# acerbilab/gpyreg

Hardware: AMD Instinct MI355X
Metric: GP-fits/sec (NLL+grad, N=4096 D=10) (higher is better)
Workload: dtype f64

## Files before the change

gpyreg_amd/_lib.py:

```python

from __future__ import annotations

import ctypes as C
import os
import threading

import numpy as np

_HERE = os.path.dirname(os.path.abspath(__file__))
LIB_PATH = os.environ.get("GPYREG_AMD_LIB") or os.path.join(_HERE, "lib", "libgpcore.so")

K_SE, K_MATERN, K_RQ, K_SE_ISO, K_MATERN_ISO = range(5)
F64, F32 = 0, 1
KLO_ZERO, KLO_ROW, KLO_COL = 0, 1, 2
KHI_FULL, KHI_ROW, KHI_COL = 0, 1, 2

_dp = C.c_void_p
_ip = C.c_void_p
_vp = C.c_void_p
_dpp = C.POINTER(C.c_double)

SIGNATURES = {
    "gpc_create": (C.c_int, [C.c_int, C.POINTER(_vp)]),
    "gpc_destroy": (None, [_vp]),
# ... 334 lines not shown
    @_serial
    def last_lauum_timing(self):
        a, b = C.c_double(), C.c_double()
        self._lib.gpc_last_lauum_timing(self._h, C.byref(a), C.byref(b))
        return a.value, b.value

    @_serial
    def mfma_peak(self, dtype=F64):
        t, cyc, ghz = C.c_double(), C.c_double(), C.c_double()
        rc = self._lib.gpc_mfma_peak(self._h, dtype, C.byref(t), C.byref(cyc), C.byref(ghz))
        self._check(rc, "gpc_mfma_peak")
        return t.value, cyc.value, ghz.value

    @_serial
    def debug_gemm(self, A, B, Cm, M, N, K, a_kmajor, b_kmajor, alpha=1.0, beta=0, klo=0, khi=0,
                   lower_only=False, dtype=F64, force_bt=0):
        A, B = _f64(A), _f64(B)
        Cm = _f64(Cm).copy()
        flags = int(bool(lower_only)) | {0: 0, 64: 0x100, 128: 0x200, 12864: 0x400}[force_bt]
        rc = self._lib.gpc_debug_gemm(self._h, dtype, M, N, K, int(a_kmajor), int(b_kmajor),
                                      float(alpha), int(beta), klo, khi, flags, _ptr(A),
                                      _ptr(B), _ptr(Cm))
        self._check(rc, "gpc_debug_gemm")
        return Cm

    @_serial
    def debug_factor(self, A, want_inv=True, dtype=F64):
        A = _f64(A)
        n = A.shape[0]
        L, W = np.empty((n, n)), np.empty((n, n))
        Ainv = np.empty((n, n)) if want_inv else None
        logdet = C.c_double()
        info = C.c_int()
        rc = self._lib.gpc_debug_factor(self._h, dtype, n, _ptr(A), _ptr(L), _ptr(W), _ptr(Ainv),
# ... 295 lines not shown
```

gpyreg_amd/csrc/gemm.h:

```cpp
#pragma once
#include "common.h"

#include <type_traits>

namespace gpc {

template <typename T>
constexpr int BKT_v = sizeof(T) == 4 ? 32 : 16;
template <typename T>
constexpr bool MM_SWZ = sizeof(T) == 4;
template <typename T>
constexpr int LDQ_v = MM_SWZ<T> ? BKT_v<T> : BKT_v<T> + 1;
constexpr int ldp_of(int BT) { return BT + 16; }
template <typename T>
constexpr int opsz_of(int BT) {
  return BKT_v<T> * (BT + 16) > BT * LDQ_v<T> ? BKT_v<T> * (BT + 16) : BT * LDQ_v<T>;
}

enum { KLO_ZERO = 0, KLO_ROW = 1, KLO_COL = 2 };
enum { KHI_FULL = 0, KHI_ROW = 1, KHI_COL = 2 };

struct GemmArgs {
  const void* A;
  const void* B;
  void* C;
  long long sA, sB, sC;
  int lda, ldb, ldc;
  int M, N, K;
  double alpha;
  int beta;
  int klo, khi, lower_only;
  int tiles_m, tiles_n;
  int flags = 0;
  const unsigned short* rsv = nullptr;
  int* ctr = nullptr;
  int ntiles = 0, batch = 0;
  double* colsq = nullptr;
  const double* ep_w = nullptr;
  long long ep_sw = 0;
  const double* ep_alpha = nullptr;
};
inline int g_gemm_flags = 8 | 16;

template <typename T, bool KM, int BT, int NT>
__device__ __forceinline__ unsigned stage_toff(int ld, int t) {
  constexpr int VEC = MM<T>::VEC;
  if constexpr (!KM) {
    constexpr int TPR = BKT_v<T> / VEC;
    return (unsigned)(t / TPR) * (unsigned)ld + (unsigned)((t % TPR) * VEC);
  } else {
    constexpr int VPR = BT / VEC;
    return (unsigned)(t / VPR) * (unsigned)ld + (unsigned)((t % VPR) * VEC);
  }
}
template <typename T, bool KM, int BT, int NT>
__device__ __forceinline__ size_t stage_pstride(int ld) {
// ... 460 lines not shown
    if (nsq <= 0) continue;
    const int total = ((g.ntiles - cls + nclass - 1) / nclass) * nsq;
    for (;;) {
      if (threadIdx.x == 0) next_tile = atomicAdd(g.ctr + q, 1);
      __syncthreads();
      const int idx = __builtin_amdgcn_readfirstlane(next_tile);
      __syncthreads();
      if (idx >= total) break;
      const int ntq = total / nsq;
      const int sq = idx / ntq, tq = idx - sq * ntq;
      gemm_tile<T, AKM, BKM, BT, NW, 0, EPI>(g, cls + tq * nclass, smp + NQ * sq, smem);
    }
  }
}

inline int g_persist_spare = 0;
inline long long g_gemm_launches = 0;
inline int g_block_slots = 512;
template <typename T, int BT, int NW>
inline hipError_t launch_gemm_bt(hipStream_t st, GemmArgs g, bool akm, bool bkm, int batch, int* ctr = nullptr,
                                 const unsigned short* reserve = nullptr) {
  const int tm = g.M / BT, tn = g.N / BT;
  g.tiles_m = tm;
  g.tiles_n = tn;
  g.flags = g_gemm_flags;
  const int ntiles = g.lower_only ? tm * (tm + 1) / 2 : tm * tn;
  if (ntiles <= 0 || batch <= 0) return hipSuccess;
  ++g_gemm_launches;
  g.ntiles = ntiles;
  g.batch = batch;
  g.ctr = ctr;
  const unsigned dyn = 0u;
  const int cap = (BT == 128 ? g_block_slots : 2 * g_block_slots) - g_persist_spare;
  g.rsv = reserve;
  if (ctr && (BT == 128 || reserve) && cap > 0 && ((long long)ntiles * batch > cap || reserve)) {
    dim3 grid(reserve ? (BT == 128 ? cap + 96 : cap) : cap), block(64 * NW);
    if (!akm && !bkm)
      hipLaunchKernelGGL((gemm_persist_kernel<T, false, false, BT, NW>), grid, block, dyn, st, g);
    else if (!akm && bkm)
      hipLaunchKernelGGL((gemm_persist_kernel<T, false, true, BT, NW>), grid, block, dyn, st, g);
    else if (akm && bkm)
      hipLaunchKernelGGL((gemm_persist_kernel<T, true, true, BT, NW>), grid, block, dyn, st, g);
    else
      hipLaunchKernelGGL((gemm_persist_kernel<T, true, false, BT, NW>), grid, block, dyn, st, g);
    return hipGetLastError();
  }
  dim3 grid(ntiles, batch), block(64 * NW);
  if (!akm && !bkm)
    hipLaunchKernelGGL((gemm_kernel<T, false, false, BT, NW>), grid, block, dyn, st, g);
  else if (!akm && bkm)
    hipLaunchKernelGGL((gemm_kernel<T, false, true, BT, NW>), grid, block, dyn, st, g);
  else if (akm && bkm)
    hipLaunchKernelGGL((gemm_kernel<T, true, true, BT, NW>), grid, block, dyn, st, g);
  else
    hipLaunchKernelGGL((gemm_kernel<T, true, false, BT, NW>), grid, block, dyn, st, g);
  return hipGetLastError();
}

#ifdef GPC_EXPERIMENTS
template <typename T>
inline hipError_t launch_gemm_rect(hipStream_t st, GemmArgs g, bool akm, bool bkm, int batch) {
  constexpr int BT = 128, BTN = 64;
// ... 78 lines not shown
  constexpr int BT = 64;
  int n[2];
  GemmArgs* gs[2] = {&g1, &g2};
  for (int i = 0; i < 2; ++i) {
    GemmArgs& g = *gs[i];
    g.tiles_m = g.M / BT;
    g.tiles_n = g.N / BT;
    g.flags = g_gemm_flags;
    g.ntiles = n[i] = g.lower_only ? g.tiles_m * (g.tiles_m + 1) / 2 : g.tiles_m * g.tiles_n;
    g.batch = batch;
    g.ctr = nullptr;
    g.rsv = nullptr;
  }
  if (n[0] + n[1] <= 0 || batch <= 0) return hipSuccess;
  ++g_gemm_launches;
  hipLaunchKernelGGL((gemm_dual_kernel<T, false, false, false, true, BT, 4>), dim3(n[0] + n[1], batch), dim3(256), 0, st,
                     g1, g2, n[0]);
  return hipGetLastError();
}

template <typename T>
inline hipError_t launch_gemm_colsq(hipStream_t st, GemmArgs g, int batch, int* ctr) {
  constexpr int BT = 128;
  g.tiles_m = g.M / BT;
  g.tiles_n = g.N / BT;
  g.flags = g_gemm_flags;
  g.lower_only = 0;
  g.ntiles = g.tiles_m * g.tiles_n;
  if (g.ntiles <= 0 || batch <= 0) return hipSuccess;
  ++g_gemm_launches;
// ... 44 lines not shown
```

gpyreg_amd/csrc/gpcore.hip:

```cpp
#include "../../include/gpcore.h"

#include <algorithm>
#include <atomic>
#include <chrono>
#include <cmath>
#include <cstdlib>
#include <cstring>
#include <memory>
#include <mutex>

#include "blas1.h"
#include "block_append.h"
#include "common.h"
#include "covfun.h"
#include "draw.h"
#include "gemm.h"
#include "leaf.h"
#include "lookahead.h"
#include "plan.h"
#include "quad.h"
#include "quad_mix.h"
#ifdef GPC_EXPERIMENTS
#include "dag.h"
#endif
// ... 2877 lines not shown
  g.A = c->dbg1.p;
  g.B = c->dbg2.p;
  g.C = c->dbg3.p;
  g.sA = g.sB = g.sC = 0;
  g.lda = akm ? M : K;
  g.ldb = bkm ? N : K;
  g.ldc = N;
  g.M = M;
  g.N = N;
  g.K = K;
  g.alpha = alpha;
  g.beta = beta;
  g.klo = klo;
  g.khi = khi;
  g.lower_only = lower & 1;
  g.tiles_n = N / TILE;
  HIPCHK(c, launch_gemm<T>(c->st, g, akm != 0, bkm != 0, 1, (lower & 0x100) ? 64 : ((lower & 0x200) ? 128 : ((lower & 0x400) ? 12864 : 0))));
  return download_as<T>(c, c->dbg3.as<T>(), C, (size_t)M * N);
}

template <typename T>
int debug_factor_impl(gpc_ctx* c, int n, const double* A, double* L, double* W, double* Ainv,
                      double* logdet, int* info) {
  const int npad = pad_tile(n);
  const size_t msz = (size_t)npad * npad;
  HIPCHK(c, c->mA.ensure(msz * sizeof(T)));
  HIPCHK(c, c->mW.ensure(msz * sizeof(T)));
  HIPCHK(c, c->mT.ensure(msz * sizeof(T)));
  HIPCHK(c, c->dbg1.ensure((size_t)n * n * 8));
  HIPCHK(c, c->scal.ensure(64));
  HIPCHK(c, hipMemcpyAsync(c->dbg1.p, A, (size_t)n * n * 8, hipMemcpyHostToDevice, c->st));
  HIPCHK(c, hipMemsetAsync(c->scal.p, 0, 64, c->st));
// ... 872 lines not shown
    g_create_err = "probing the CU map failed: " + c->err;
    delete c;
    return -1;
  }
  if (const char* e = getenv("GPC_LEAF")) gpc::g_leaf_version = atoi(e) == 3 ? 3 : 5;
  if (const char* e = getenv("GPC_SMALL_PATH")) c->small_path = atoi(e) != 0;
  if (const char* e = getenv("GPC_GRAPH_MAX_NPAD")) c->graph_max_npad = atoi(e);
#ifdef GPC_EXPERIMENTS
  if (const char* e = getenv("GPC_RL_PANEL")) c->rl_panel = atoi(e) <= 0 ? 0 : std::max(TILE, (atoi(e) / TILE) * TILE);
  if (const char* e = getenv("GPC_RECT_MIN")) gpc::g_rect_min_blocks = atoi(e);
#endif
  if (const char* e = getenv("GPC_NLL_BLOCK")) c->nll_block = atoi(e) < 0 ? -1 : (atoi(e) == 0 ? 0 : std::max(TILE, (atoi(e) / TILE) * TILE));
  if (const char* e = getenv("GPC_GROUPS")) c->groups = std::max(1, std::min((int)gpc_ctx::MAXG, atoi(e)));
  if (const char* e = getenv("GPC_SMALL_BLOCKS")) gpc::g_small_launch_blocks = atoi(e);
  if (const char* e = getenv("GPC_DUAL")) gpc::g_dual_launch = atoi(e) != 0;
  if (const char* e = getenv("GPC_GEMM_FLAGS")) gpc::g_gemm_flags = atoi(e);
  if (const char* e = getenv("GPC_XCD_AFFINE")) gpc::g_gemm_flags = atoi(e) ? (gpc::g_gemm_flags | 8) : (gpc::g_gemm_flags & ~8);
  *out = c;
  return 0;
}

void gpc_destroy(gpc_ctx* c) {
  if (!c) return;
  (void)hipSetDevice(c->device);
  (void)hipStreamSynchronize(c->st);
  DevBuf* bufs[] = {&c->dX,   &c->dY,  &c->mA,    &c->mW,  &c->mT,   &c->xs,   &c->spb,  &c->mulb, &c->divb,
                    &c->dvec, &c->rvec,  &c->zvec, &c->avec, &c->scal, &c->parts, &c->gout, &c->diagq,
                    &c->dmb,  &c->dsn2b, &c->mg,  &c->ng,   &c->ks,   &c->vb,   &c->xss,  &c->pout, &c->kss,
                    &c->dbg1, &c->dbg2,  &c->dbg3, &c->tpart, &c->qb, &c->gpart, &c->gres, &c->qcon, &c->qmix, &c->zb, &c->fb, &c->dout, &c->daux, &c->tile_ctr, &c->rsv_tbl};
  for (auto& g : c->graphs)
// ... 634 lines not shown
  if (n == "dag_timeout_ms") return std::max(1, value);
  return value;
}
#endif
}

int gpc_set_option(gpc_ctx* c, const char* name, int value) {
  if (!c || !name) return -2;
  const std::string n(name);
  if (n == "groups")
    c->groups = std::max(1, std::min((int)gpc_ctx::MAXG, value));
  else if (n == "small_blocks")
    gpc::g_small_launch_blocks = value;
  else if (n == "dual_launch")
    gpc::g_dual_launch = value != 0;
  else if (n == "leaf")
    gpc::g_leaf_version = value == 3 ? 3 : 5;
  else if (n == "defer_min")
    c->defer_min = value;
  else if (n == "defer_reserve") {
    c->defer_reserve = value;
    if (build_reserve_table(c)) return -1;
  } else if (n == "leaf_fault")
    gpc::g_leaf_fault = value != 0;
  else if (n == "nll_block")
    c->nll_block = value < 0 ? -1 : (value == 0 ? 0 : std::max(TILE, (value / TILE) * TILE));
  else if (n == "solves_beside_lauum")
    c->solves_beside_lauum = value != 0;
  else if (n == "stable")
    c->stable = value != 0;
// ... 17 lines not shown
      *slot = clamp_experiment_option(n, value);
    else
#endif
      FAIL(c, "gpc_set_option: unknown option");
  }
  ++g_alloc_epoch;
  return 0;
}

int gpc_get_option(gpc_ctx* c, const char* name, int* value) {
  if (!c || !name || !value) return -2;
  const std::string n(name);
  if (n == "groups") *value = c->groups;
  else if (n == "small_blocks") *value = gpc::g_small_launch_blocks;
  else if (n == "dual_launch") *value = gpc::g_dual_launch ? 1 : 0;
  else if (n == "leaf") *value = gpc::g_leaf_version;
  else if (n == "defer_min") *value = c->defer_min;
  else if (n == "defer_reserve") *value = c->defer_reserve;
  else if (n == "nll_block") *value = c->nll_block;
  else if (n == "solves_beside_lauum") *value = c->solves_beside_lauum;
  else if (n == "stable") *value = c->stable;
  else if (n == "small_path") *value = c->small_path;
  else if (n == "check_queues") *value = c->check_queues;
  else if (n == "small_poll") *value = c->small_poll;
  else if (n == "small_timing") *value = c->small_timing;
  else if (n == "small_polled") *value = (int)(c->small_polled & 0x7fffffff);
  else if (n == "small_synced") *value = (int)(c->small_synced & 0x7fffffff);
  else if (n == "cov_fused") *value = (int)(c->cov_fused & 0x7fffffff);
  else if (n == "quad_mix_gemms") *value = (int)(c->quad_mix_gemms & 0x7fffffff);
  else if (n == "block_engine") *value = c->block_engine;
// ... 100 lines not shown
        best_cyc = best_ghz * 1e9 * (4.0 * prop.multiProcessorCount) * (2.0 * 16 * 16 * 4) / (tf * 1e12);
      }
    }
  *tflops = best;
  if (cycles_per_mfma) *cycles_per_mfma = best_cyc;
  if (clock_ghz) *clock_ghz = best_ghz;
  return 0;
}


int gpc_debug_gemm(gpc_ctx* c, int dtype, int M, int N, int K, int a_kmajor, int b_kmajor, double alpha,
                   int beta, int klo, int khi, int lower_only, const double* A, const double* B, double* C) {
  if (!c) return -2;
  if (M % TILE || N % TILE || K % TILE || M <= 0 || N <= 0 || K <= 0) FAIL(c, "gpc_debug_gemm: sizes must be multiples of 128");
  if ((lower_only & 1) && M != N) FAIL(c, "gpc_debug_gemm: lower_only needs M == N");
#ifndef GPC_EXPERIMENTS
  if (lower_only & 0x400) FAIL(c, "gpc_debug_gemm: the rectangular tile exists in the experiments build only");
#endif
  HIPCHK(c, hipSetDevice(c->device));
  return dtype == GPC_F64
             ? debug_gemm_impl<double>(c, M, N, K, a_kmajor, b_kmajor, alpha, beta, klo, khi, lower_only, A, B, C)
             : debug_gemm_impl<float>(c, M, N, K, a_kmajor, b_kmajor, alpha, beta, klo, khi, lower_only, A, B, C);
}

int gpc_debug_leaf(gpc_ctx* c, int dtype, const double* A, double* L, double* W, double* logdet, int* info) {
  return gpc_debug_factor(c, dtype, TILE, A, L, W, nullptr, logdet, info);
}

int gpc_debug_factor(gpc_ctx* c, int dtype, int n, const double* A, double* L, double* W, double* Ainv,
                     double* logdet, int* info) {
// ... 112 lines not shown
```

gpyreg_amd/csrc/plan.h:

```cpp
#pragma once
#include "blas1.h"
#include "gemm.h"
#include "leaf.h"

#include <algorithm>

namespace gpc {

#ifdef GPC_EXPERIMENTS
struct PlanRecorder {
  struct Op {
    int kind;
    GemmArgs g;
    bool akm, bkm;
    int off;
  };
  std::vector<Op> ops;
  bool unsupported = false;
};
#endif

template <typename T>
struct Factor {
#ifdef GPC_EXPERIMENTS
// ... 36 lines not shown
  hipEvent_t ev_tail = nullptr;
  int tail_row0 = 1 << 30;
  void need_rows(int hi) {
    if (ev_tail && hi > tail_row0) {
      chk(hipStreamWaitEvent(st, ev_tail, 0));
      ev_tail = nullptr;
    }
  }
  double flops = 0;
  int launches = 0;
  hipError_t err = hipSuccess;

  T* blk(T* base, int r, int c) const { return base + (size_t)r * npad + c; }

  GemmArgs make_args(T* C, long long sC, const T* Aop, long long sAop, const T* Bop, long long sBop, int M, int N,
                     int K, double alpha, int beta, int klo, int khi, int lower) {
    GemmArgs g;
    g.A = Aop;
    g.B = Bop;
    g.C = C;
    g.sA = sAop;
    g.sB = sBop;
    g.sC = sC;
    g.lda = g.ldb = g.ldc = npad;
    g.M = M;
    g.N = N;
    g.K = K;
    g.alpha = alpha;
    g.beta = beta;
    g.klo = klo;
    g.khi = khi;
    g.lower_only = lower;
    g.tiles_n = N / TILE;
    flops += gemm_flops(g, batch);
    return g;
  }

  void gemm(T* C, long long sC, const T* Aop, long long sAop, const T* Bop, long long sBop, int M,
            int N, int K, bool akm, bool bkm, double alpha, int beta, int klo, int khi, int lower,
            hipStream_t on = nullptr, const unsigned short* rsv = nullptr) {
    GemmArgs g;
    g.A = Aop;
    g.B = Bop;
    g.C = C;
    g.sA = sAop;
    g.sB = sBop;
    g.sC = sC;
    g.lda = g.ldb = g.ldc = npad;
    g.M = M;
    g.N = N;
    g.K = K;
    g.alpha = alpha;
    g.beta = beta;
    g.klo = klo;
    g.khi = khi;
    g.lower_only = lower;
    g.tiles_n = N / TILE;
    flops += gemm_flops(g, batch);
    ++launches;
#ifdef GPC_EXPERIMENTS
    if (rec) {
      rec->ops.push_back({0, g, akm, bkm, 0});
      return;
    }
#endif
    int* slot = nullptr;
    const long long tm = M / TILE, tn = N / TILE;
    const long long blocks128 = (lower ? tm * (tm + 1) / 2 : tm * tn) * batch;
    if (!rsv && reserve_all && reserve && blocks128 >= reserve_min) rsv = reserve;
    const bool persistent = rsv || (blocks128 >= g_small_launch_blocks && blocks128 > g_block_slots - g_persist_spare);
    if (persistent && ctr && ctr_used + CTR_STRIDE <= ctr_cap) {
// ... 22 lines not shown
      }
#endif
      need_rows(off + TILE);
      launch_leaf<T>(st, batch, blk(A, off, off), sA, npad, blk(W, off, off), sW, npad, off, logdet, info,
                     std::max(0, std::min(TILE, nvalid - off)), stable);
      flops += (2.0 / 3.0) * TILE * (double)TILE * TILE * batch;
      ++launches;
      return;
    }
    const int q = n / TILE;
    const int n1 = (q / 2) * TILE, n2 = n - n1;
    const int o1 = off, o2 = off + n1;
    potrf_inv(o1, n1, true, keep_L);
    need_rows(o2 + n2);
    gemm(blk(Tm, o2, o1), sT, blk(A, o2, o1), sA, blk(W, o1, o1), sW, n2, n1, n1, false, false, 1.0,
         0, KLO_ZERO, KHI_COL, 0);
    if (stable) {
      gemm(blk(A, o2, o1), sA, blk(Tm, o2, o1), sT, blk(A, o1, o1), sA, n2, n1, n1, false, false, -1.0, 1, KLO_ZERO,
           KHI_COL, 0);
      gemm(blk(Tm, o2, o1), sT, blk(A, o2, o1), sA, blk(W, o1, o1), sW, n2, n1, n1, false, false, 1.0, 1, KLO_ZERO,
           KHI_COL, 0);
    }
    const bool defer = need_inv && side && defer_min > 0 && n >= defer_min && ev_used + 2 <= nev;
    bool u_done = false;
    {
      GemmArgs gs = make_args(blk(A, o2, o2), sA, blk(Tm, o2, o1), sT, blk(Tm, o2, o1), sT, n2, n2, n1, -1.0, 1,
                              KLO_ZERO, KHI_FULL, 1);
      const long long syrk_tiles = (long long)(n2 / TILE) * (n2 / TILE + 1) / 2 * batch;
      if (need_inv && !defer && dual_launch && !rec && gemm_is_small(gs, batch) && !(reserve_all && syrk_tiles >= reserve_min)) {
        GemmArgs gu = make_args(blk(A, o2, o1), sA, blk(Tm, o2, o1), sT, blk(W, o1, o1), sW, n2, n1, n1, 1.0, 0,
                                KLO_COL, KHI_FULL, 0);
        if (gemm_is_small(gu, batch)) {
          hipError_t e = launch_gemm_dual_small<T>(st, gs, gu, batch);
          if (e != hipSuccess && err == hipSuccess) err = e;
          ++launches;
          u_done = true;
        } else {
          flops -= gemm_flops(gu, batch);
        }
      }
      if (!u_done) {
        flops -= gemm_flops(gs, batch);
        gemm(blk(A, o2, o2), sA, blk(Tm, o2, o1), sT, blk(Tm, o2, o1), sT, n2, n2, n1, false, false, -1.0, 1,
             KLO_ZERO, KHI_FULL, 1);
      }
    }
    hipEvent_t ev_join = nullptr;
    if (defer) {
      hipEvent_t ev_fork = evs[ev_used++];
      ev_join = evs[ev_used++];
      chk(hipEventRecord(ev_fork, st));
      chk(hipStreamWaitEvent(side, ev_fork, 0));
      gemm(blk(A, o2, o1), sA, blk(Tm, o2, o1), sT, blk(W, o1, o1), sW, n2, n1, n1, false, true, 1.0, 0,
           KLO_COL, KHI_FULL, 0, side, reserve);
      chk(hipEventRecord(ev_join, side));
    }
    potrf_inv(o2, n2, need_inv, keep_L);
    if (need_inv) {
      if (defer)
        chk(hipStreamWaitEvent(st, ev_join, 0));
      else if (!u_done)
        gemm(blk(A, o2, o1), sA, blk(Tm, o2, o1), sT, blk(W, o1, o1), sW, n2, n1, n1, false, true, 1.0, 0,
             KLO_COL, KHI_FULL, 0);
      gemm(blk(W, o2, o1), sW, blk(W, o2, o2), sW, blk(A, o2, o1), sA, n2, n1, n2, false, true, -1.0,
           0, KLO_ZERO, KHI_ROW, 0);
    }
#ifdef GPC_EXPERIMENTS
    if (keep_L && rec) rec->unsupported = true;
#endif
    if (keep_L && !rec) {
      dim3 grid((n1 + 64 * MM<T>::VEC - 1) / (64 * MM<T>::VEC), n2 / 32, batch), block(64, 4);
      hipLaunchKernelGGL((rect_copy_kernel<T>), grid, block, 0, st, (const T*)blk(Tm, o2, o1), sT, npad,
                         blk(A, o2, o1), sA, npad, n2, n1);
      ++launches;
    }
  }

  int nll_block = 0;

  void trsm_nll(int r0, int m, int c0, int n) {
    if (n <= nll_block) {
      gemm(blk(Tm, r0, c0), sT, blk(A, r0, c0), sA, blk(W, c0, c0), sW, m, n, n, false, false, 1.0, 0, KLO_ZERO,
           KHI_COL, 0);
      if (stable) {
        gemm(blk(A, r0, c0), sA, blk(Tm, r0, c0), sT, blk(A, c0, c0), sA, m, n, n, false, false, -1.0, 1, KLO_ZERO,
             KHI_COL, 0);
        gemm(blk(Tm, r0, c0), sT, blk(A, r0, c0), sA, blk(W, c0, c0), sW, m, n, n, false, false, 1.0, 1, KLO_ZERO,
             KHI_COL, 0);
      }
      return;
    }
    const int q = n / TILE;
    const int n1 = (q / 2) * TILE, n2 = n - n1;
    trsm_nll(r0, m, c0, n1);
    gemm(blk(A, r0, c0 + n1), sA, blk(Tm, r0, c0), sT, blk(Tm, c0 + n1, c0), sT, m, n2, n1, false, false, -1.0, 1,
         KLO_ZERO, KHI_FULL, 0);
    trsm_nll(r0, m, c0 + n1, n2);
  }

  void potrf_nll(int off, int n) {
    if (n <= nll_block || n == TILE) {
      potrf_inv(off, n, true, false);
      return;
    }
    const int q = n / TILE;
    const int n1 = (q / 2) * TILE, n2 = n - n1;
    const int o1 = off, o2 = off + n1;
    potrf_nll(o1, n1);
    need_rows(o2 + n2);
    trsm_nll(o2, n2, o1, n1);
    gemm(blk(A, o2, o2), sA, blk(Tm, o2, o1), sT, blk(Tm, o2, o1), sT, n2, n2, n1, false, false, -1.0, 1, KLO_ZERO,
         KHI_FULL, 1);
    potrf_nll(o2, n2);
  }

  void forward_solve_nll(int off, int n, double* r, double* z) {
    if (n <= nll_block || n == TILE) {
      hipLaunchKernelGGL((trmv_kernel<T>), dim3(n / 4, batch), dim3(256), 0, st, (const T*)W, sW, npad,
                         (const double*)r, npad, z, off);
      ++launches;
      return;
    }
    const int q = n / TILE;
    const int n1 = (q / 2) * TILE, n2 = n - n1;
    forward_solve_nll(off, n1, r, z);
    hipLaunchKernelGGL((gemv_sub_kernel<T>), dim3(n2 / 4, batch), dim3(256), 0, st, (const T*)Tm, sT, npad,
                       (const double*)z, r, npad, off + n1, off, n1);
// ... 67 lines not shown
        hipLaunchKernelGGL((trmv_kernel<T>), dim3(n / 4, batch), dim3(256), 0, st, (const T*)W, sW, npad,
                           (const double*)r, npad, z, off);
      ++launches;
      return;
    }
    const int q = n / TILE;
    const int n1 = (q / 2) * TILE, n2 = n - n1;
    forward_solve(off, n1, true, r, z);
    hipLaunchKernelGGL((gemv_sub_kernel<T>), dim3(n2 / 4, batch), dim3(256), 0, st, (const T*)Tm, sT, npad,
                       (const double*)z, r, npad, off + n1, off, n1);
    ++launches;
    forward_solve(off + n1, n2, need_inv, r, z);
  }

  void lauum(T* out, long long sOut) {
    gemm(out, sOut, W, sW, W, sW, npad, npad, npad, true, true, 1.0, 0, KLO_ROW, KHI_FULL, 1);
  }
};

}
```

Before: 839.5.

## Add triangle-aware GEMM kernels that skip zero MFMA blocks in edge slabs

```diff
diff --git a/gpyreg_amd/_lib.py b/gpyreg_amd/_lib.py
--- a/gpyreg_amd/_lib.py
+++ b/gpyreg_amd/_lib.py
@@ -372,10 +372,11 @@
 
     @_serial
     def debug_gemm(self, A, B, Cm, M, N, K, a_kmajor, b_kmajor, alpha=1.0, beta=0, klo=0, khi=0,
-                   lower_only=False, dtype=F64, force_bt=0):
+                   lower_only=False, dtype=F64, force_bt=0, tri=0, batch=1):
         A, B = _f64(A), _f64(B)
         Cm = _f64(Cm).copy()
         flags = int(bool(lower_only)) | {0: 0, 64: 0x100, 128: 0x200, 12864: 0x400}[force_bt]
+        flags |= (int(tri) & 15) << 12 | (int(batch) & 0xff) << 16
         rc = self._lib.gpc_debug_gemm(self._h, dtype, M, N, K, int(a_kmajor), int(b_kmajor),
                                       float(alpha), int(beta), klo, khi, flags, _ptr(A),
                                       _ptr(B), _ptr(Cm))
diff --git a/gpyreg_amd/csrc/gemm.h b/gpyreg_amd/csrc/gemm.h
--- a/gpyreg_amd/csrc/gemm.h
+++ b/gpyreg_amd/csrc/gemm.h
@@ -19,6 +19,7 @@
 
 enum { KLO_ZERO = 0, KLO_ROW = 1, KLO_COL = 2 };
 enum { KHI_FULL = 0, KHI_ROW = 1, KHI_COL = 2 };
+enum { TRI_NONE = 0, TRI_A_FIRST = 1, TRI_A_LAST = 2, TRI_B_FIRST = 3, TRI_B_LAST = 4, TRI_OPND = 7, TRI_SYM = 8 };
 
 struct GemmArgs {
   const void* A;
@@ -39,7 +40,9 @@
   const double* ep_w = nullptr;
   long long ep_sw = 0;
   const double* ep_alpha = nullptr;
+  int tri = TRI_NONE;
 };
+inline int g_tri_skip = 1;
 inline int g_gemm_flags = 8 | 16;
 
 template <typename T, bool KM, int BT, int NT>
@@ -530,6 +533,373 @@
   }
 }
 
+template <int ILO, int IHI, int JLO, int JHI, bool DG = false>
+struct Live {
+  static constexpr int ilo = ILO, ihi = IHI, jlo = JLO, jhi = JHI;
+  static constexpr bool on(int i, int j) { return i >= ILO && i < IHI && j >= JLO && j < JHI && (!DG || i >= j); }
+  static constexpr int count() {
+    int n = 0;
+    for (int i = ILO; i < IHI; ++i)
+      for (int j = JLO; j < JHI; ++j) n += on(i, j) ? 1 : 0;
+    return n;
+  }
+};
+
+template <bool AKM, bool BKM, int BT, int TRI, bool DG>
+__device__ __forceinline__ void gemm_tile_tri_at(const GemmArgs& g, const int ti, const int tj, const int by,
+                                                 double* __restrict__ smem) {
+  using T = double;
+  using acc_t = typename MM<T>::acc_t;
+  using vec_t = typename MM<T>::vec_t;
+  constexpr int NT = 256, BK = BKT_v<T>;
+  constexpr int NV = (BT * BK) / (NT * MM<T>::VEC);
+  constexpr int OPSZ = opsz_of<T>(BT), STG = 2 * OPSZ;
+  constexpr int MR = BT / 32;
+  constexpr int TOP = TRI & TRI_OPND;
+  static_assert(TRI != TRI_NONE && NV >= 1 && MR >= 2 && (!DG || (TRI & TRI_SYM)), "tile shape");
+  const int t = threadIdx.x;
+  const int lane = t & 63, w = t >> 6, wr = w >> 1, wc = w & 1;
+  const int m0 = ti * BT, n0 = tj * BT;
+  int k0 = g.klo == KLO_ROW ? m0 : (g.klo == KLO_COL ? n0 : 0);
+  int k1 = g.khi == KHI_ROW ? m0 + BT : (g.khi == KHI_COL ? n0 + BT : g.K);
+  if (k1 > g.K) k1 = g.K;
+  const int nk = (k1 - k0) / BK;
+
+  const T* __restrict__ A = reinterpret_cast<const T*>(g.A) + (size_t)by * g.sA;
+  const T* __restrict__ B = reinterpret_cast<const T*>(g.B) + (size_t)by * g.sB;
+  T* __restrict__ C = reinterpret_cast<T*>(g.C) + (size_t)by * g.sC;
+
+  acc_t acc[MR][MR];
+#pragma unroll
+  for (int i = 0; i < MR; ++i)
+#pragma unroll
+    for (int j = 0; j < MR; ++j) acc[i][j] = acc_t{0, 0, 0, 0};
+
+  if (nk > 0) {
+    vec_t ra[NV], rb[NV];
+    const unsigned toa = stage_toff<T, AKM, BT, NT>(g.lda, t) * (unsigned)sizeof(T),
+                   tob = stage_toff<T, BKM, BT, NT>(g.ldb, t) * (unsigned)sizeof(T);
+    const unsigned psa = (unsigned)(stage_pstride<T, AKM, BT, NT>(g.lda) * sizeof(T)),
+                   psb = (unsigned)(stage_pstride<T, BKM, BT, NT>(g.ldb) * sizeof(T));
+    const T* pa = AKM ? A + (size_t)k0 * g.lda + m0 : A + (size_t)m0 * g.lda + k0;
+    const T* pb = BKM ? B + (size_t)k0 * g.ldb + n0 : B + (size_t)n0 * g.ldb + k0;
+    const size_t rowsa = (size_t)BK * g.lda, rowsb = (size_t)BK * g.ldb;
+    __amdgpu_buffer_rsrc_t rsa = make_rsrc(pa), rsb = make_rsrc(pb);
+    unsigned ua = 0, ub = 0;
+    auto next_slab = [&]() {
+      if constexpr (AKM) {
+        pa += rowsa;
+        rsa = make_rsrc(pa);
+      } else {
+        ua += (unsigned)(BK * sizeof(T));
+      }
+      if constexpr (BKM) {
+        pb += rowsb;
+        rsb = make_rsrc(pb);
+      } else {
+        ub += (unsigned)(BK * sizeof(T));
+      }
+    };
+    g2r<T, AKM, BT, NT>(ra, rsa, ua, psa, toa);
+    g2r<T, BKM, BT, NT>(rb, rsb, ub, psb, tob);
+    r2s<T, AKM, BT, NT>(smem, ra, t);
+    r2s<T, BKM, BT, NT>(smem + OPSZ, rb, t);
+    next_slab();
+    g2r<T, AKM, BT, NT>(ra, rsa, ua, psa, toa);
+    g2r<T, BKM, BT, NT>(rb, rsb, ub, psb, tob);
+    __syncthreads();
+
+    T af[2][MR], bf[2][MR];
+    auto load_frags = [&](int set, const T* a_s, const T* b_s, int kk) {
+#pragma unroll
+      for (int i = 0; i < MR; ++i)
+        af[set][i] = frag<T, AKM, BT>(a_s, (wr + 2 * i) * 16, kk, lane);
+#pragma unroll
+      for (int j = 0; j < MR; ++j)
+        bf[set][j] = frag<T, BKM, BT>(b_s, (wc + 2 * j) * 16, kk, lane);
+    };
+    auto mfmas = [&](int set, auto lv) {
+      using LV = decltype(lv);
+#pragma unroll
+      for (int i = 0; i < MR; ++i)
+#pragma unroll
+        for (int j = 0; j < MR; ++j)
+          if (LV::on(i, j)) acc[i][j] = MM<T>::mma(af[set][i], bf[set][j], acc[i][j]);
+    };
+    constexpr int NMEM = 2 * NV;
+    constexpr int KS = BK / 4;
+    auto slab = [&](auto cur_c, auto wr_c, auto ld_c, auto lv) {
+      using LV = decltype(lv);
+      constexpr int CUR = decltype(cur_c)::value;
+      constexpr bool WR = decltype(wr_c)::value, LD = decltype(ld_c)::value;
+      constexpr int NM = LV::count();
+      constexpr int NFR = 2 * MR;
+      constexpr int PER = NM / NMEM, REM = NM - PER * NMEM;
+      constexpr int MPER = NM >= NMEM ? 0 : (NMEM + NM - 1) / NM;
+      static_assert(NM >= 1, "a slab with no live block is not issued");
+      const T* a_s = smem + CUR * STG;
+      const T* b_s = a_s + OPSZ;
+      T* a_n = smem + (CUR ^ 1) * STG;
+#pragma unroll
+      for (int ks = 0; ks < KS - 2; ++ks) {
+        load_frags((ks + 1) & 1, a_s, b_s, 4 * (ks + 1));
+        mfmas(ks & 1, lv);
+        __builtin_amdgcn_sched_group_barrier(0x100, NFR, 0);
+        __builtin_amdgcn_sched_group_barrier(0x008, NM, 0);
+      }
+      load_frags(1, a_s, b_s, 4 * (KS - 1));
+      mfmas(0, lv);
+      if constexpr (WR) {
+        r2s<T, AKM, BT, NT>(a_n, ra, t);
+        r2s<T, BKM, BT, NT>(a_n + OPSZ, rb, t);
+      }
+      __builtin_amdgcn_sched_group_barrier(0x100, NFR, 0);
+      if constexpr (NM >= NMEM) {
+#pragma unroll
+        for (int q = 0; q < NMEM; ++q) {
+          __builtin_amdgcn_sched_group_barrier(0x008, PER, 0);
+          if constexpr (WR) __builtin_amdgcn_sched_group_barrier(0x200, 1, 0);
+        }
+        if constexpr (REM > 0) __builtin_amdgcn_sched_group_barrier(0x008, REM, 0);
+      } else {
+#pragma unroll
+        for (int q = 0; q < NM; ++q) {
+          __builtin_amdgcn_sched_group_barrier(0x008, 1, 0);
+          if constexpr (WR) __builtin_amdgcn_sched_group_barrier(0x200, MPER, 0);
+        }
+      }
+      __syncthreads();
+      if constexpr (LD) {
+        next_slab();
+        g2r<T, AKM, BT, NT>(ra, rsa, ua, psa, toa);
+        g2r<T, BKM, BT, NT>(rb, rsb, ub, psb, tob);
+      }
+      if constexpr (WR) load_frags(0, a_n, a_n + OPSZ, 0);
+      mfmas(1, lv);
+      if constexpr (WR) __builtin_amdgcn_sched_group_barrier(0x100, NFR, 0);
+      if constexpr (NM >= NMEM) {
+#pragma unroll
+        for (int q = 0; q < NMEM; ++q) {
+          __builtin_amdgcn_sched_group_barrier(0x008, PER, 0);
+          if constexpr (LD) __builtin_amdgcn_sched_group_barrier(0x020, 1, 0);
+        }
+        if constexpr (REM > 0) __builtin_amdgcn_sched_group_barrier(0x008, REM, 0);
+      } else {
+#pragma unroll
+        for (int q = 0; q < NM; ++q) {
+          __builtin_amdgcn_sched_group_barrier(0x008, 1, 0);
+          if constexpr (LD) __builtin_amdgcn_sched_group_barrier(0x020, MPER, 0);
+        }
+      }
+    };
+    using I0 = std::integral_constant<int, 0>;
+    using I1 = std::integral_constant<int, 1>;
+    using Yes = std::true_type;
+    using No = std::false_type;
+    load_frags(0, smem, smem + OPSZ, 0);
+    constexpr int NP = BT / BK - 2;
+    constexpr bool FIRST = TOP == TRI_A_FIRST || TOP == TRI_B_FIRST, LAST = TOP == TRI_A_LAST || TOP == TRI_B_LAST;
+    constexpr bool ONA = TOP == TRI_A_FIRST || TOP == TRI_A_LAST;
+    using FullD = Live<0, MR, 0, MR, DG>;
+    {
+      auto peeled = [&](auto s_c, auto wr_c, auto ld_c) {
+        constexpr int S = decltype(s_c)::value;
+        constexpr int LO = FIRST ? 0 : (S + 2) / 2, HI = FIRST ? S / 2 + 1 : MR;
+        static_assert(LO < HI && HI <= MR, "live range of a peeled slab");
+        using LV = std::conditional_t<ONA, Live<LO, HI, 0, MR, DG>, Live<0, MR, LO, HI, DG>>;
+        slab(std::integral_constant<int, (S & 1)>{}, wr_c, ld_c, LV{});
+      };
+      int it = 0;
+      if constexpr (FIRST) {
+        peeled(std::integral_constant<int, 0>{}, Yes{}, Yes{});
+        peeled(std::integral_constant<int, 1>{}, Yes{}, Yes{});
+        if constexpr (NP > 2) {
+          peeled(std::integral_constant<int, 2>{}, Yes{}, Yes{});
+          peeled(std::integral_constant<int, 3>{}, Yes{}, Yes{});
+          peeled(std::integral_constant<int, 4>{}, Yes{}, Yes{});
+          peeled(std::integral_constant<int, 5>{}, Yes{}, Yes{});
+        }
+        it = NP;
+      }
+      constexpr int TAIL = LAST ? NP : 2;
+      for (; it + TAIL + 1 < nk; it += 2) {
+        slab(I0{}, Yes{}, Yes{}, FullD{});
+        slab(I1{}, Yes{}, Yes{}, FullD{});
+      }
+      if constexpr (LAST) {
+        if constexpr (NP > 2) {
+          peeled(std::integral_constant<int, 0>{}, Yes{}, Yes{});
+          peeled(std::integral_constant<int, 1>{}, Yes{}, Yes{});
+          peeled(std::integral_constant<int, 2>{}, Yes{}, Yes{});
+          peeled(std::integral_constant<int, 3>{}, Yes{}, Yes{});
+        }
+        peeled(std::integral_constant<int, NP - 2>{}, Yes{}, No{});
+        peeled(std::integral_constant<int, NP - 1>{}, No{}, No{});
+      } else {
+        slab(I0{}, Yes{}, No{}, FullD{});
+        slab(I1{}, No{}, No{}, FullD{});
+      }
+    }
+  }
+
+  if constexpr (DG) {
+    {
+      constexpr int NSL = MR * (MR - 1) / 2, SLOT = 16 * 17;
+      static_assert(4 * NSL * SLOT <= 2 * STG, "the mirror slots fit the LDS stages");
+      __syncthreads();
+#pragma unroll
+      for (int i = 0; i < MR; ++i)
+#pragma unroll
+        for (int j = 0; j < MR; ++j)
+          if (i > j) {
+            T* sl = smem + (w * NSL + i * (i - 1) / 2 + j) * SLOT;
+#pragma unroll
+            for (int r = 0; r < 4; ++r) sl[MM<T>::row_of(lane, r) * 17 + (lane & 15)] = acc[i][j][r];
+          }
+      __syncthreads();
+#pragma unroll
+      for (int i = 0; i < MR; ++i)
+#pragma unroll
+        for (int j = 0; j < MR; ++j)
+          if (i < j) {
+            const T* sl = smem + ((wc * 2 + wr) * NSL + j * (j - 1) / 2 + i) * SLOT;
+#pragma unroll
+            for (int r = 0; r < 4; ++r) acc[i][j][r] = sl[(lane & 15) * 17 + MM<T>::row_of(lane, r)];
+          }
+      __syncthreads();
+    }
+  }
+  const T alpha = (T)g.alpha;
+#pragma unroll
+  for (int i = 0; i < MR; ++i) {
+    T old[MR][4];
+    if (g.beta) {
+#pragma unroll
+      for (int j = 0; j < MR; ++j)
+#pragma unroll
+        for (int r = 0; r < 4; ++r) {
+          const int row = m0 + (wr + 2 * i) * 16 + MM<T>::row_of(lane, r);
+          const int col = n0 + (wc + 2 * j) * 16 + (lane & 15);
+          old[j][r] = C[(size_t)row * g.ldc + col];
+        }
+    }
+#pragma unroll
+    for (int j = 0; j < MR; ++j)
+#pragma unroll
+      for (int r = 0; r < 4; ++r) {
+        const int row = m0 + (wr + 2 * i) * 16 + MM<T>::row_of(lane, r);
+        const int col = n0 + (wc + 2 * j) * 16 + (lane & 15);
+        T v = alpha * acc[i][j][r];
+        if (g.beta) v += old[j][r];
+        C[(size_t)row * g.ldc + col] = v;
+      }
+  }
+}
+
+template <bool AKM, bool BKM, int BT, int TRI>
+__device__ __forceinline__ void gemm_tile_tri(const GemmArgs& g, const int bx, const int by, double* __restrict__ smem) {
+  int ti, tj;
+  if (g.lower_only) {
+    tri_tile(bx, ti, tj);
+  } else if (g.khi == KHI_COL) {
+    tj = g.tiles_n - 1 - bx / g.tiles_m;
+    ti = bx % g.tiles_m;
+  } else if (g.klo == KLO_COL) {
+    tj = bx / g.tiles_m;
+    ti = bx % g.tiles_m;
+  } else if (g.khi == KHI_ROW) {
+    ti = g.tiles_m - 1 - bx / g.tiles_n;
+    tj = bx % g.tiles_n;
+  } else {
+    ti = bx / g.tiles_n;
+    tj = bx % g.tiles_n;
+  }
+  if constexpr ((TRI & TRI_SYM) != 0) {
+    if (ti == tj) {
+      gemm_tile_tri_at<AKM, BKM, BT, TRI, true>(g, ti, tj, by, smem);
+      return;
+    }
+  }
+  gemm_tile_tri_at<AKM, BKM, BT, TRI, false>(g, ti, tj, by, smem);
+}
+
+template <bool AKM, bool BKM, int BT, int TRI>
+__global__ __launch_bounds__(256, 2) void gemm_tri_kernel(GemmArgs g) {
+  __shared__ __attribute__((aligned(16))) double smem[4 * opsz_of<double>(BT)];
+  int bx = blockIdx.x, by = blockIdx.y;
+  if ((g.flags & 16) && gridDim.y >= 8) {
+    const int total = gridDim.x * gridDim.y, per = total >> 3;
+    const int L = blockIdx.y * gridDim.x + blockIdx.x;
+    if (L < (per << 3)) {
+      const int wk = (L & 7) * per + (L >> 3);
+      bx = wk % (int)gridDim.x;
+      by = wk / (int)gridDim.x;
+    }
+  }
+  gemm_tile_tri<AKM, BKM, BT, TRI>(g, bx, by, smem);
+}
+template <int BT>
+__global__ __launch_bounds__(256, 2) void gemm_tri_dual_kernel(GemmArgs g1, GemmArgs g2, int n1) {
+  __shared__ __attribute__((aligned(16))) double smem[4 * opsz_of<double>(BT)];
+  int bx = blockIdx.x, by = blockIdx.y;
+  if ((g1.flags & 16) && gridDim.y >= 8) {
+    const int total = gridDim.x * gridDim.y, per = total >> 3;
+    const int L = blockIdx.y * gridDim.x + blockIdx.x;
+    if (L < (per << 3)) {
+      const int wk = (L & 7) * per + (L >> 3);
+      bx = wk % (int)gridDim.x;
+      by = wk / (int)gridDim.x;
+    }
+  }
+  if (bx < n1)
+    gemm_tile_tri<false, false, BT, TRI_SYM>(g1, bx, by, smem);
+  else
+    gemm_tile_tri<false, true, BT, TRI_B_FIRST>(g2, bx - n1, by, smem);
+}
+template <bool AKM, bool BKM, int BT, int TRI>
+__global__ __launch_bounds__(256, 2) void gemm_tri_persist_kernel(GemmArgs g) {
+  __shared__ __attribute__((aligned(16))) double smem[4 * opsz_of<double>(BT)];
+  __shared__ int next_tile;
+  if (g.rsv && cu_reserve_bail(g.rsv, g.ctr)) return;
+  unsigned xcc;
+  asm volatile("s_getreg_b32 %0, hwreg(HW_REG_XCC_ID)" : "=s"(xcc));
+  const int q0 = (int)(xcc & (NQ - 1));
+  const int nclass = g.batch >= NQ ? 1 : NQ / g.batch;
+  for (int a = 0; a < NQ; ++a) {
+    const int q = (q0 + a) & (NQ - 1);
+    int nsq, cls = 0, smp = q;
+    if (g.batch >= NQ) {
+      nsq = (g.batch - q + NQ - 1) / NQ;
+    } else {
+      if (q >= g.batch * nclass) continue;
+      nsq = 1;
+      smp = q % g.batch;
+      cls = q / g.batch;
+    }
+    if (nsq <= 0) continue;
+    const int total = ((g.ntiles - cls + nclass - 1) / nclass) * nsq;
+    for (;;) {
+      if (threadIdx.x == 0) next_tile = atomicAdd(g.ctr + q, 1);
+      __syncthreads();
+      const int idx = __builtin_amdgcn_readfirstlane(next_tile);
+      __syncthreads();
+      if (idx >= total) break;
+      const int ntq = total / nsq;
+      const int sq = idx / ntq, tq = idx - sq * ntq;
+      gemm_tile_tri<AKM, BKM, BT, TRI>(g, cls + tq * nclass, smp + NQ * sq, smem);
+    }
+  }
+}
+
+inline bool tri_mode_known(bool akm, bool bkm, const GemmArgs& g) {
+  const int tri = g.tri, top = tri & TRI_OPND;
+  if ((top == TRI_A_FIRST && g.klo != KLO_ROW) || (top == TRI_A_LAST && g.khi != KHI_ROW) ||
+      (top == TRI_B_FIRST && g.klo != KLO_COL) || (top == TRI_B_LAST && g.khi != KHI_COL))
+    return false;
+  if ((tri & TRI_SYM) && (!g.lower_only || g.M != g.N)) return false;
+  return (!akm && !bkm && (tri == TRI_B_LAST || tri == TRI_SYM)) || (!akm && bkm && (tri == TRI_B_FIRST || tri == TRI_A_LAST)) ||
+         (akm && bkm && tri == (TRI_A_FIRST | TRI_SYM));
+}
 inline int g_persist_spare = 0;
 inline long long g_gemm_launches = 0;
 inline int g_block_slots = 512;
@@ -540,6 +910,7 @@
   g.tiles_m = tm;
   g.tiles_n = tn;
   g.flags = g_gemm_flags;
+  if (sizeof(T) != 8 || NW != 4 || !g_tri_skip || !tri_mode_known(akm, bkm, g)) g.tri = TRI_NONE;
   const int ntiles = g.lower_only ? tm * (tm + 1) / 2 : tm * tn;
   if (ntiles <= 0 || batch <= 0) return hipSuccess;
   ++g_gemm_launches;
@@ -551,6 +922,22 @@
   g.rsv = reserve;
   if (ctr && (BT == 128 || reserve) && cap > 0 && ((long long)ntiles * batch > cap || reserve)) {
     dim3 grid(reserve ? (BT == 128 ? cap + 96 : cap) : cap), block(64 * NW);
+    if constexpr (BT == 128) {
+      if (g.tri == (TRI_A_FIRST | TRI_SYM)) g.tri = TRI_A_FIRST;
+      if (g.tri && (g.flags & 8)) {
+        if (!akm && !bkm && g.tri == TRI_B_LAST)
+          hipLaunchKernelGGL((gemm_tri_persist_kernel<false, false, BT, TRI_B_LAST>), grid, block, 0, st, g);
+        else if (!akm && !bkm)
+          hipLaunchKernelGGL((gemm_tri_persist_kernel<false, false, BT, TRI_SYM>), grid, block, 0, st, g);
+        else if (!akm && bkm && g.tri == TRI_B_FIRST)
+          hipLaunchKernelGGL((gemm_tri_persist_kernel<false, true, BT, TRI_B_FIRST>), grid, block, 0, st, g);
+        else if (!akm && bkm)
+          hipLaunchKernelGGL((gemm_tri_persist_kernel<false, true, BT, TRI_A_LAST>), grid, block, 0, st, g);
+        else
+          hipLaunchKernelGGL((gemm_tri_persist_kernel<true, true, BT, TRI_A_FIRST>), grid, block, 0, st, g);
+        return hipGetLastError();
+      }
+    }
     if (!akm && !bkm)
       hipLaunchKernelGGL((gemm_persist_kernel<T, false, false, BT, NW>), grid, block, dyn, st, g);
     else if (!akm && bkm)
@@ -562,6 +949,19 @@
     return hipGetLastError();
   }
   dim3 grid(ntiles, batch), block(64 * NW);
+  if (g.tri) {
+    if (!akm && !bkm && g.tri == TRI_B_LAST)
+      hipLaunchKernelGGL((gemm_tri_kernel<false, false, BT, TRI_B_LAST>), grid, block, 0, st, g);
+    else if (!akm && !bkm)
+      hipLaunchKernelGGL((gemm_tri_kernel<false, false, BT, TRI_SYM>), grid, block, 0, st, g);
+    else if (!akm && bkm && g.tri == TRI_B_FIRST)
+      hipLaunchKernelGGL((gemm_tri_kernel<false, true, BT, TRI_B_FIRST>), grid, block, 0, st, g);
+    else if (!akm && bkm)
+      hipLaunchKernelGGL((gemm_tri_kernel<false, true, BT, TRI_A_LAST>), grid, block, 0, st, g);
+    else
+      hipLaunchKernelGGL((gemm_tri_kernel<true, true, BT, TRI_A_FIRST | TRI_SYM>), grid, block, 0, st, g);
+    return hipGetLastError();
+  }
   if (!akm && !bkm)
     hipLaunchKernelGGL((gemm_kernel<T, false, false, BT, NW>), grid, block, dyn, st, g);
   else if (!akm && bkm)
@@ -670,6 +1070,11 @@
   }
   if (n[0] + n[1] <= 0 || batch <= 0) return hipSuccess;
   ++g_gemm_launches;
+  if (sizeof(T) == 8 && g_tri_skip && g1.tri == TRI_SYM && g2.tri == TRI_B_FIRST && tri_mode_known(false, false, g1) &&
+      tri_mode_known(false, true, g2)) {
+    hipLaunchKernelGGL((gemm_tri_dual_kernel<BT>), dim3(n[0] + n[1], batch), dim3(256), 0, st, g1, g2, n[0]);
+    return hipGetLastError();
+  }
   hipLaunchKernelGGL((gemm_dual_kernel<T, false, false, false, true, BT, 4>), dim3(n[0] + n[1], batch), dim3(256), 0, st,
                      g1, g2, n[0]);
   return hipGetLastError();
diff --git a/gpyreg_amd/csrc/gpcore.hip b/gpyreg_amd/csrc/gpcore.hip
--- a/gpyreg_amd/csrc/gpcore.hip
+++ b/gpyreg_amd/csrc/gpcore.hip
@@ -2915,8 +2915,15 @@
   g.klo = klo;
   g.khi = khi;
   g.lower_only = lower & 1;
+  g.tri = (lower >> 12) & 15;
   g.tiles_n = N / TILE;
-  HIPCHK(c, launch_gemm<T>(c->st, g, akm != 0, bkm != 0, 1, (lower & 0x100) ? 64 : ((lower & 0x200) ? 128 : ((lower & 0x400) ? 12864 : 0))));
+  const int batch = std::max(1, (lower >> 16) & 0xff);
+  int* ctr = nullptr;
+  if (batch > 1) {
+    ctr = c->tile_ctr.as<int>() + (size_t)gpc_ctx::MAXG * gpc_ctx::CTR_PER_GROUP;
+    HIPCHK(c, hipMemsetAsync(ctr, 0, CTR_STRIDE * sizeof(int), c->st));
+  }
+  HIPCHK(c, launch_gemm<T>(c->st, g, akm != 0, bkm != 0, batch, (lower & 0x100) ? 64 : ((lower & 0x200) ? 128 : ((lower & 0x400) ? 12864 : 0)), ctr));
   return download_as<T>(c, c->dbg3.as<T>(), C, (size_t)M * N);
 }
 
@@ -3819,6 +3826,7 @@
   if (const char* e = getenv("GPC_GROUPS")) c->groups = std::max(1, std::min((int)gpc_ctx::MAXG, atoi(e)));
   if (const char* e = getenv("GPC_SMALL_BLOCKS")) gpc::g_small_launch_blocks = atoi(e);
   if (const char* e = getenv("GPC_DUAL")) gpc::g_dual_launch = atoi(e) != 0;
+  if (const char* e = getenv("GPC_TRI_SKIP")) gpc::g_tri_skip = atoi(e) != 0;
   if (const char* e = getenv("GPC_GEMM_FLAGS")) gpc::g_gemm_flags = atoi(e);
   if (const char* e = getenv("GPC_XCD_AFFINE")) gpc::g_gemm_flags = atoi(e) ? (gpc::g_gemm_flags | 8) : (gpc::g_gemm_flags & ~8);
   *out = c;
@@ -4483,6 +4491,8 @@
     gpc::g_small_launch_blocks = value;
   else if (n == "dual_launch")
     gpc::g_dual_launch = value != 0;
+  else if (n == "tri_skip")
+    gpc::g_tri_skip = value != 0;
   else if (n == "leaf")
     gpc::g_leaf_version = value == 3 ? 3 : 5;
   else if (n == "defer_min")
@@ -4530,6 +4540,7 @@
   if (n == "groups") *value = c->groups;
   else if (n == "small_blocks") *value = gpc::g_small_launch_blocks;
   else if (n == "dual_launch") *value = gpc::g_dual_launch ? 1 : 0;
+  else if (n == "tri_skip") *value = gpc::g_tri_skip ? 1 : 0;
   else if (n == "leaf") *value = gpc::g_leaf_version;
   else if (n == "defer_min") *value = c->defer_min;
   else if (n == "defer_reserve") *value = c->defer_reserve;
@@ -4660,6 +4671,7 @@
   if (!c) return -2;
   if (M % TILE || N % TILE || K % TILE || M <= 0 || N <= 0 || K <= 0) FAIL(c, "gpc_debug_gemm: sizes must be multiples of 128");
   if ((lower_only & 1) && M != N) FAIL(c, "gpc_debug_gemm: lower_only needs M == N");
+  if (((lower_only >> 16) & 0xff) > 1 && beta != 0) FAIL(c, "gpc_debug_gemm: a batch count needs beta == 0");
 #ifndef GPC_EXPERIMENTS
   if (lower_only & 0x400) FAIL(c, "gpc_debug_gemm: the rectangular tile exists in the experiments build only");
 #endif
diff --git a/gpyreg_amd/csrc/plan.h b/gpyreg_amd/csrc/plan.h
--- a/gpyreg_amd/csrc/plan.h
+++ b/gpyreg_amd/csrc/plan.h
@@ -74,7 +74,7 @@
   T* blk(T* base, int r, int c) const { return base + (size_t)r * npad + c; }
 
   GemmArgs make_args(T* C, long long sC, const T* Aop, long long sAop, const T* Bop, long long sBop, int M, int N,
-                     int K, double alpha, int beta, int klo, int khi, int lower) {
+                     int K, double alpha, int beta, int klo, int khi, int lower, int tri = TRI_NONE) {
     GemmArgs g;
     g.A = Aop;
     g.B = Bop;
@@ -91,6 +91,7 @@
     g.klo = klo;
     g.khi = khi;
     g.lower_only = lower;
+    g.tri = tri;
     g.tiles_n = N / TILE;
     flops += gemm_flops(g, batch);
     return g;
@@ -98,7 +99,7 @@
 
   void gemm(T* C, long long sC, const T* Aop, long long sAop, const T* Bop, long long sBop, int M,
             int N, int K, bool akm, bool bkm, double alpha, int beta, int klo, int khi, int lower,
-            hipStream_t on = nullptr, const unsigned short* rsv = nullptr) {
+            hipStream_t on = nullptr, const unsigned short* rsv = nullptr, int tri = TRI_NONE) {
     GemmArgs g;
     g.A = Aop;
     g.B = Bop;
@@ -115,6 +116,7 @@
     g.klo = klo;
     g.khi = khi;
     g.lower_only = lower;
+    g.tri = tri;
     g.tiles_n = N / TILE;
     flops += gemm_flops(g, batch);
     ++launches;
@@ -167,22 +169,22 @@
     potrf_inv(o1, n1, true, keep_L);
     need_rows(o2 + n2);
     gemm(blk(Tm, o2, o1), sT, blk(A, o2, o1), sA, blk(W, o1, o1), sW, n2, n1, n1, false, false, 1.0,
-         0, KLO_ZERO, KHI_COL, 0);
+         0, KLO_ZERO, KHI_COL, 0, nullptr, nullptr, TRI_B_LAST);
     if (stable) {
       gemm(blk(A, o2, o1), sA, blk(Tm, o2, o1), sT, blk(A, o1, o1), sA, n2, n1, n1, false, false, -1.0, 1, KLO_ZERO,
            KHI_COL, 0);
       gemm(blk(Tm, o2, o1), sT, blk(A, o2, o1), sA, blk(W, o1, o1), sW, n2, n1, n1, false, false, 1.0, 1, KLO_ZERO,
-           KHI_COL, 0);
+           KHI_COL, 0, nullptr, nullptr, TRI_B_LAST);
     }
     const bool defer = need_inv && side && defer_min > 0 && n >= defer_min && ev_used + 2 <= nev;
     bool u_done = false;
     {
       GemmArgs gs = make_args(blk(A, o2, o2), sA, blk(Tm, o2, o1), sT, blk(Tm, o2, o1), sT, n2, n2, n1, -1.0, 1,
-                              KLO_ZERO, KHI_FULL, 1);
+                              KLO_ZERO, KHI_FULL, 1, TRI_SYM);
       const long long syrk_tiles = (long long)(n2 / TILE) * (n2 / TILE + 1) / 2 * batch;
       if (need_inv && !defer && dual_launch && !rec && gemm_is_small(gs, batch) && !(reserve_all && syrk_tiles >= reserve_min)) {
         GemmArgs gu = make_args(blk(A, o2, o1), sA, blk(Tm, o2, o1), sT, blk(W, o1, o1), sW, n2, n1, n1, 1.0, 0,
-                                KLO_COL, KHI_FULL, 0);
+                                KLO_COL, KHI_FULL, 0, TRI_B_FIRST);
         if (gemm_is_small(gu, batch)) {
           hipError_t e = launch_gemm_dual_small<T>(st, gs, gu, batch);
           if (e != hipSuccess && err == hipSuccess) err = e;
@@ -195,7 +197,7 @@
       if (!u_done) {
         flops -= gemm_flops(gs, batch);
         gemm(blk(A, o2, o2), sA, blk(Tm, o2, o1), sT, blk(Tm, o2, o1), sT, n2, n2, n1, false, false, -1.0, 1,
-             KLO_ZERO, KHI_FULL, 1);
+             KLO_ZERO, KHI_FULL, 1, nullptr, nullptr, TRI_SYM);
       }
     }
     hipEvent_t ev_join = nullptr;
@@ -205,7 +207,7 @@
       chk(hipEventRecord(ev_fork, st));
       chk(hipStreamWaitEvent(side, ev_fork, 0));
       gemm(blk(A, o2, o1), sA, blk(Tm, o2, o1), sT, blk(W, o1, o1), sW, n2, n1, n1, false, true, 1.0, 0,
-           KLO_COL, KHI_FULL, 0, side, reserve);
+           KLO_COL, KHI_FULL, 0, side, reserve, TRI_B_FIRST);
       chk(hipEventRecord(ev_join, side));
     }
     potrf_inv(o2, n2, need_inv, keep_L);
@@ -214,9 +216,9 @@
         chk(hipStreamWaitEvent(st, ev_join, 0));
       else if (!u_done)
         gemm(blk(A, o2, o1), sA, blk(Tm, o2, o1), sT, blk(W, o1, o1), sW, n2, n1, n1, false, true, 1.0, 0,
-             KLO_COL, KHI_FULL, 0);
+             KLO_COL, KHI_FULL, 0, nullptr, nullptr, TRI_B_FIRST);
       gemm(blk(W, o2, o1), sW, blk(W, o2, o2), sW, blk(A, o2, o1), sA, n2, n1, n2, false, true, -1.0,
-           0, KLO_ZERO, KHI_ROW, 0);
+           0, KLO_ZERO, KHI_ROW, 0, nullptr, nullptr, TRI_A_LAST);
     }
 #ifdef GPC_EXPERIMENTS
     if (keep_L && rec) rec->unsupported = true;
@@ -234,12 +236,12 @@
   void trsm_nll(int r0, int m, int c0, int n) {
     if (n <= nll_block) {
       gemm(blk(Tm, r0, c0), sT, blk(A, r0, c0), sA, blk(W, c0, c0), sW, m, n, n, false, false, 1.0, 0, KLO_ZERO,
-           KHI_COL, 0);
+           KHI_COL, 0, nullptr, nullptr, TRI_B_LAST);
       if (stable) {
         gemm(blk(A, r0, c0), sA, blk(Tm, r0, c0), sT, blk(A, c0, c0), sA, m, n, n, false, false, -1.0, 1, KLO_ZERO,
              KHI_COL, 0);
         gemm(blk(Tm, r0, c0), sT, blk(A, r0, c0), sA, blk(W, c0, c0), sW, m, n, n, false, false, 1.0, 1, KLO_ZERO,
-             KHI_COL, 0);
+             KHI_COL, 0, nullptr, nullptr, TRI_B_LAST);
       }
       return;
     }
@@ -263,7 +265,7 @@
     need_rows(o2 + n2);
     trsm_nll(o2, n2, o1, n1);
     gemm(blk(A, o2, o2), sA, blk(Tm, o2, o1), sT, blk(Tm, o2, o1), sT, n2, n2, n1, false, false, -1.0, 1, KLO_ZERO,
-         KHI_FULL, 1);
+         KHI_FULL, 1, nullptr, nullptr, TRI_SYM);
     potrf_nll(o2, n2);
   }
 
@@ -361,7 +363,8 @@
   }
 
   void lauum(T* out, long long sOut) {
-    gemm(out, sOut, W, sW, W, sW, npad, npad, npad, true, true, 1.0, 0, KLO_ROW, KHI_FULL, 1);
+    gemm(out, sOut, W, sW, W, sW, npad, npad, npad, true, true, 1.0, 0, KLO_ROW, KHI_FULL, 1, nullptr, nullptr,
+         TRI_A_FIRST | TRI_SYM);
   }
 };
 
```

After: 855.0, median of 6. 1.8% higher.
